# icdm-adteam/MoCoPCI

Hardware: AMD Instinct MI355X
Metric: interpolated frames/sec (higher is better)
Workload: dtype f32 (fused MLP layers: fp32 products as 6 bf16-MFMA partials of an exact 3-way split, fp32 accumulate; index paths exact f32)

## Files before the change

### mocopci_amd/csrc/cross.hip

```cpp
#include "common.h"
#include "cross_tile.h"

#ifdef MCP_CROSS_DIAG
__device__ unsigned long long g_cross_diag[8];
#define CROSS_STAMP(slot)                                                                            \
    do {                                                                                             \
        unsigned long long t_;                                                                       \
        __builtin_amdgcn_sched_barrier(0);                                                           \
        asm volatile("s_memtime %0\n\ts_waitcnt lgkmcnt(0)" : "=s"(t_)::"memory");                   \
        __builtin_amdgcn_sched_barrier(0);                                                           \
        if (blockIdx.x == 0 && blockIdx.y == 0 && threadIdx.x == 0) g_cross_diag[slot] += t_ - t_prev; \
        t_prev = t_;                                                                                 \
    } while (0)
#else
#define CROSS_STAMP(slot)
#endif

namespace {

constexpr int MAX_MAPPED_BATCH = 1024;

template <int CTRL>
__device__ __forceinline__ float dppf(float v) {
    return __uint_as_float(mcp_dpp<CTRL>(__float_as_uint(v)));
}
#define MCP_MAX_DPP(dst, src0, src1, CTRL)                                                                              \
    asm("s_nop 1\n\tv_max_f32_dpp %0, %1, %2 " CTRL : "+v"(dst) : "v"(src0), "v"(src1))

__device__ __forceinline__ float scatter_max(const f32x16 &acc, int lane) {
    float v8[8], v4[4], v2[2];
#pragma unroll
    for (int r = 0; r < 8; ++r) {
        const auto sw = __builtin_amdgcn_permlane16_swap(__float_as_uint(acc[r]), __float_as_uint(acc[r + 8]), false, false);
        const float a = __uint_as_float(sw[0]), b = __uint_as_float(sw[1]);
        asm("v_max_f32 %0, %1, %2" : "=v"(v8[r]) : "v"(a), "v"(b));
    }
#pragma unroll
    for (int r = 0; r < 4; ++r) {
        float d = v8[r + 4];
        MCP_MAX_DPP(d, v8[r], v8[r], "row_ror:8 row_mask:0xf bank_mask:0x3");
        MCP_MAX_DPP(d, v8[r + 4], d, "row_ror:8 row_mask:0xf bank_mask:0xc");
        v4[r] = d;
    }
#pragma unroll
    for (int r = 0; r < 2; ++r) {
        float d = v4[r + 2];
        MCP_MAX_DPP(d, v4[r], v4[r], "row_half_mirror row_mask:0xf bank_mask:0x5");
        MCP_MAX_DPP(d, v4[r + 2], d, "row_half_mirror row_mask:0xf bank_mask:0xa");
        v2[r] = d;
    }
    const bool b1 = (lane & 2) != 0;
    float keep = b1 ? v2[1] : v2[0];
    const float send = b1 ? v2[0] : v2[1];
    MCP_MAX_DPP(keep, send, keep, "quad_perm:[2,3,0,1] row_mask:0xf bank_mask:0xf");
    MCP_MAX_DPP(keep, keep, keep, "quad_perm:[1,0,3,2] row_mask:0xf bank_mask:0xf");
    return keep;
}
__device__ __forceinline__ int scatter_reg(int lane) { return ((lane >> 4) & 1) * 8 + ((lane >> 3) & 1) * 4 + ((lane >> 2) & 1) * 2 + ((lane >> 1) & 1); }

template <int D>
__global__ __launch_bounds__(256) void cross_pack_kernel(const float *__restrict__ wpos, const float *__restrict__ bpos,
                                                         const float *__restrict__ wmlp, const float *__restrict__ bmlp,
                                                         float *__restrict__ packed) {
    using L = CrossLds<D>;
    for (int e = blockIdx.x * 256 + threadIdx.x; e < L::FLOATS; e += gridDim.x * 256) {
        float v;
        if (e < L::OFF_POS) continue;
        else if (e < L::OFF_B) {
            const int f = e - L::OFF_POS, lane = f & 63, s = (f >> 6) & 1, t = f >> 7;
            const int row = 32 * t + (lane & 31), c = 2 * s + (lane >> 5);
            v = c < 3 ? wpos[row * 3 + c] : bpos[row];
        } else {
            const int f = e - L::OFF_B, r = f & 15, h = (f >> 4) & 1, t = f >> 5;
            v = bmlp[32 * t + mcp_chan_of(r, h)];
        }
        packed[e] = v;
    }
    mcp_split_weights(reinterpret_cast<uint4 *>(packed + L::OFF_W), wmlp, D, L::T, blockIdx.x * 256 + threadIdx.x, gridDim.x * 256);
}

template <int D>
struct CrossShape {
    static constexpr int NW = D == 128 ? 8 : 4;
    static constexpr int WG_PER_CU = D == 64 ? 3 : 1;
    static constexpr int GRID = D == 64 ? 768 : 256;
};

template <int D, int SPLIT>
__global__ __launch_bounds__(64 * CrossShape<D>::NW, CrossShape<D>::WG_PER_CU) void cross_kernel(long long total, int n1, int n2, const float *__restrict__ xyz1,
                                                           const float *__restrict__ xyz2, const float *__restrict__ points1,
                                                           const float *__restrict__ points2, const int *__restrict__ idx,
                                                           const int *__restrict__ idx2, const int *__restrict__ bmap, int shared,
                                                           const float *__restrict__ packed, float *__restrict__ out) {
    using L = CrossLds<D>;
    constexpr int T = L::T;
    constexpr int WAVES = CrossShape<D>::NW;
    constexpr int TO = T / SPLIT;
    constexpr int WH = L::W_FLOATS / SPLIT, SMALL = L::POS_FLOATS + L::B_FLOATS;
    extern __shared__ __attribute__((aligned(16))) float lds[];
    const int tid = threadIdx.x, split = blockIdx.y;
    static_assert(WH % 4 == 0 && SMALL % 4 == 0, "LDS image is copied as float4");
    for (int e = tid; e < WH / 4; e += 64 * WAVES)
        reinterpret_cast<float4 *>(lds)[e] = reinterpret_cast<const float4 *>(packed + L::OFF_W + (size_t)split * WH)[e];
    for (int e = tid; e < SMALL / 4; e += 64 * WAVES)
        reinterpret_cast<float4 *>(lds + WH)[e] = reinterpret_cast<const float4 *>(packed + L::OFF_POS)[e];
    if (bmap) {
        const int nb = (int)(total / n1);
        for (int e = tid; e < nb; e += 64 * WAVES) reinterpret_cast<int *>(lds + WH + SMALL + WAVES * D)[e] = bmap[e];
    }
    __syncthreads();

    const int lane = tid & 63, wave = tid >> 6, h = lane >> 5, col = lane & 31;
    const float *lpos = lds + WH, *lbias = lds + WH + L::POS_FLOATS;
    float *row1_lds = lds + WH + SMALL + wave * D;
    const int *bmap_lds = reinterpret_cast<const int *>(lds + WH + SMALL + WAVES * D);

#ifndef MCP_NO_XCD_MAP
    const bool by_xcd = gridDim.x >= 8 && (gridDim.x & 7) == 0;
#else
    const bool by_xcd = false;
#endif
    const long long chunk = by_xcd ? (total + 7) / 8 : total;
    const long long stride = (long long)(by_xcd ? gridDim.x >> 3 : gridDim.x) * WAVES;
    const long long limit = by_xcd ? min(total, ((long long)(blockIdx.x & 7) + 1) * chunk) : total;
    long long p = by_xcd ? (long long)(blockIdx.x & 7) * chunk + (long long)(blockIdx.x >> 3) * WAVES + wave : (long long)blockIdx.x * WAVES + wave;
    float q2x = 0.f, q2y = 0.f, q2z = 0.f, p1x = 0.f, p1y = 0.f, p1z = 0.f;
    float4 r1 = make_float4(0.f, 0.f, 0.f, 0.f);
    float4 rg[T][4];
    auto mapped = [&](int bb, int flag) -> long long { return (bmap && (shared & flag)) ? (long long)bmap_lds[bb] : (long long)bb; };
    struct Pos { int bb, off; };
    const int stride_b = (int)(stride / n1), stride_o = (int)(stride % n1);
    auto advance = [&](Pos q) {
        q.bb += stride_b;
        q.off += stride_o;
        if (q.off >= n1) { q.off -= n1; ++q.bb; }
        return q;
    };
    auto fetch = [&](long long pp, Pos q, int id) {
        const float *q2 = xyz2 + ((long long)q.bb * n2 + id) * 3;
        q2x = q2[0]; q2y = q2[1]; q2z = q2[2];
        p1x = xyz1[pp * 3 + 0]; p1y = xyz1[pp * 3 + 1]; p1z = xyz1[pp * 3 + 2];
        const float4 *row2 = reinterpret_cast<const float4 *>(points2 + (mapped(q.bb, 2) * n2 + id) * D);
        const float4 *row1 = reinterpret_cast<const float4 *>(points1 + (mapped(q.bb, 1) * n1 + q.off) * D);
        r1 = row1[lane < D / 4 ? lane : 0];
#pragma unroll
        for (int t = 0; t < T; ++t)
#pragma unroll
            for (int g = 0; g < 4; ++g) rg[t][g] = row2[(32 * t + 8 * g + 4 * h) >> 2];
    };
    auto nbr = [&](long long pp, Pos q) { return cross_nbr(idx, idx2, pp, [&] { return mapped(q.bb, 4) * n1 + q.off; }, col); };
    long long pn = p + stride;
    Pos qp{(int)(p / n1), (int)(p % n1)};
    Pos qn = advance(qp), qnn = advance(qn);
    int idn = 0;
    if (p < limit) {
        fetch(p, qp, nbr(p, qp));
        if (pn < limit) idn = nbr(pn, qn);
    }
#ifdef MCP_CROSS_DIAG
    unsigned long long t_prev = 0;
    CROSS_STAMP(7);
#endif
    for (; p < limit; p = pn, pn += stride) {
        CROSS_STAMP(0);
        McpSplit3 xs[2 * T];
        const float in0 = h ? q2y - p1y : q2x - p1x, in1 = h ? 1.0f : q2z - p1z;
        if (lane < D / 4) reinterpret_cast<float4 *>(row1_lds)[lane] = r1;
        __builtin_amdgcn_wave_barrier();
#pragma unroll
        for (int t = 0; t < T; ++t) {
            f32x16 acc;
#pragma unroll
            for (int g = 0; g < 4; ++g) {
                const float4 a = reinterpret_cast<const float4 *>(row1_lds)[(32 * t + 8 * g + 4 * h) >> 2];
                acc[4 * g + 0] = a.x; acc[4 * g + 1] = a.y; acc[4 * g + 2] = a.z; acc[4 * g + 3] = a.w;
            }
            acc = __builtin_amdgcn_mfma_f32_32x32x2f32(lpos[(t * 2 + 0) * 64 + lane], in0, acc, 0, 0, 0);
            acc = __builtin_amdgcn_mfma_f32_32x32x2f32(lpos[(t * 2 + 1) * 64 + lane], in1, acc, 0, 0, 0);
#pragma unroll
            for (int g = 0; g < 4; ++g) {
                acc[4 * g + 0] = leaky(acc[4 * g + 0] + rg[t][g].x);
                acc[4 * g + 1] = leaky(acc[4 * g + 1] + rg[t][g].y);
                acc[4 * g + 2] = leaky(acc[4 * g + 2] + rg[t][g].z);
                acc[4 * g + 3] = leaky(acc[4 * g + 3] + rg[t][g].w);
            }
            xs[2 * t + 0] = mcp_split_kstep(acc, 0);
            xs[2 * t + 1] = mcp_split_kstep(acc, 1);
        }
        __builtin_amdgcn_wave_barrier();
        CROSS_STAMP(1);
        if (pn < limit) {
            fetch(pn, qn, idn);
            if (pn + stride < limit) idn = nbr(pn + stride, qnn);
        }
        qn = qnn;
        qnn = advance(qnn);
        CROSS_STAMP(2);
#pragma unroll 1
        for (int tl = 0; tl < TO; ++tl) {
            const int t = TO * split + tl;
            f32x16 acc;
#pragma unroll
            for (int r = 0; r < 16; ++r) acc[r] = lbias[(t * 2 + h) * 16 + r];
            acc = mcp_tile_split<2 * T>(reinterpret_cast<const uint4 *>(lds) + (size_t)tl * (2 * T) * 3 * 64 + lane, xs, acc);
            CROSS_STAMP(3);
            const float m = leaky(scatter_max(acc, lane));
            if ((lane & 1) == 0) out[p * D + 32 * t + mcp_chan_of(scatter_reg(lane), h)] = m;
            CROSS_STAMP(4);
        }
    }
}

__global__ __launch_bounds__(64 * X256_WAVES, 1) void cross256_stream_kernel(long long total, int n1, int n2, const float *__restrict__ xyz1,
                                                                          const float *__restrict__ xyz2, const float *__restrict__ points1,
                                                                          const float *__restrict__ points2, const int *__restrict__ idx,
                                                                          const int *__restrict__ idx2, const int *__restrict__ bmap, int shared,
                                                                          const float *__restrict__ packed, float *__restrict__ out) {
    using L = CrossLds<256>;
    constexpr int D = 256, T = X256_T, WAVES = X256_WAVES, SMALL = L::POS_FLOATS + L::B_FLOATS;
    extern __shared__ __attribute__((aligned(16))) float lds[];
    uint4 *wbuf = reinterpret_cast<uint4 *>(lds);
    float *small = lds + 2 * X256_TILE_U4 * 4;
    float *row1_all = small + SMALL;
    int *bmap_lds = reinterpret_cast<int *>(row1_all + WAVES * D);
    const int tid = threadIdx.x, lane = tid & 63, wave = tid >> 6, h = lane >> 5, col = lane & 31;
    const uint4 *wimg = reinterpret_cast<const uint4 *>(packed + L::OFF_W);
    for (int e = tid; e < SMALL / 4; e += 64 * WAVES) reinterpret_cast<float4 *>(small)[e] = reinterpret_cast<const float4 *>(packed + L::OFF_POS)[e];
    if (bmap) {
        const int nb = (int)(total / n1);
        for (int e = tid; e < nb; e += 64 * WAVES) bmap_lds[e] = bmap[e];
    }
    for (int e = tid; e < X256_TILE_U4; e += 64 * WAVES) wbuf[e] = wimg[e];
    __syncthreads();
    const float *lpos = small, *lbias = small + L::POS_FLOATS;
    float *row1_lds = row1_all + wave * D;
    auto mapped = [&](int bb, int flag) -> long long { return (bmap && (shared & flag)) ? (long long)bmap_lds[bb] : (long long)bb; };

    const long long per_round = (long long)gridDim.x * WAVES;
    const long long first = (long long)blockIdx.x * WAVES;
    const int rounds = first < total ? (int)((total - first + per_round - 1) / per_round) : 0;
    int cur = 0;
    for (int g = 0; g < rounds; ++g) {
        const long long pw = first + (long long)g * per_round + wave;
        const bool live = pw < total;
        const long long p = live ? pw : total - 1;
        const int bb = (int)(p / n1), off = (int)(p - (long long)bb * n1);
        int id;
        if (!idx2) {
            id = idx[p * KNB + col];
        } else {
            const long long ps = mapped(bb, 4) * n1 + off;
            id = col >= 16 ? idx2[p * 16 + col - 16] : idx[ps * 16 + col];
        }
        const float *q2 = xyz2 + ((long long)bb * n2 + id) * 3;
        const float dx = q2[0] - xyz1[p * 3 + 0], dy = q2[1] - xyz1[p * 3 + 1], dz = q2[2] - xyz1[p * 3 + 2];
        const float in0 = h ? dy : dx, in1 = h ? 1.0f : dz;
        const float4 *row2 = reinterpret_cast<const float4 *>(points2 + (mapped(bb, 2) * n2 + id) * D);
        const float4 *row1 = reinterpret_cast<const float4 *>(points1 + (mapped(bb, 1) * n1 + off) * D);
        reinterpret_cast<float4 *>(row1_lds)[lane] = row1[lane];
        __builtin_amdgcn_wave_barrier();
        McpSplit3 xs[2 * T];
#pragma unroll
        for (int t = 0; t < T; ++t) {
            f32x16 acc;
            float4 rg[4];
#pragma unroll
            for (int gq = 0; gq < 4; ++gq) {
                const float4 a = reinterpret_cast<const float4 *>(row1_lds)[(32 * t + 8 * gq + 4 * h) >> 2];
                rg[gq] = row2[(32 * t + 8 * gq + 4 * h) >> 2];
                acc[4 * gq + 0] = a.x; acc[4 * gq + 1] = a.y; acc[4 * gq + 2] = a.z; acc[4 * gq + 3] = a.w;
            }
            acc = __builtin_amdgcn_mfma_f32_32x32x2f32(lpos[(t * 2 + 0) * 64 + lane], in0, acc, 0, 0, 0);
            acc = __builtin_amdgcn_mfma_f32_32x32x2f32(lpos[(t * 2 + 1) * 64 + lane], in1, acc, 0, 0, 0);
#pragma unroll
            for (int gq = 0; gq < 4; ++gq) {
                acc[4 * gq + 0] = leaky(acc[4 * gq + 0] + rg[gq].x);
                acc[4 * gq + 1] = leaky(acc[4 * gq + 1] + rg[gq].y);
                acc[4 * gq + 2] = leaky(acc[4 * gq + 2] + rg[gq].z);
                acc[4 * gq + 3] = leaky(acc[4 * gq + 3] + rg[gq].w);
            }
            xs[2 * t + 0] = mcp_split_kstep(acc, 0);
            xs[2 * t + 1] = mcp_split_kstep(acc, 1);
        }
        __builtin_amdgcn_wave_barrier();
#pragma unroll 1
        for (int t = 0; t < T; ++t) {
            const bool more = t + 1 < T || g + 1 < rounds;
            const uint4 *nsrc = wimg + (size_t)((t + 1) & (T - 1)) * X256_TILE_U4 + tid;
            uint4 nx[X256_TILE_U4 / (64 * X256_WAVES)];
#pragma unroll
            for (int i = 0; i < X256_TILE_U4 / (64 * WAVES); ++i) nx[i] = more ? nsrc[i * 64 * WAVES] : make_uint4(0u, 0u, 0u, 0u);
            f32x16 acc;
#pragma unroll
            for (int r = 0; r < 16; ++r) acc[r] = lbias[(t * 2 + h) * 16 + r];
            acc = mcp_tile_split<2 * T>(wbuf + (size_t)cur * X256_TILE_U4 + lane, xs, acc);
            const float m = leaky(scatter_max(acc, lane));
            if (live && (lane & 1) == 0) out[p * D + 32 * t + mcp_chan_of(scatter_reg(lane), h)] = m;
            uint4 *ndst = wbuf + (size_t)(cur ^ 1) * X256_TILE_U4 + tid;
#pragma unroll
            for (int i = 0; i < X256_TILE_U4 / (64 * WAVES); ++i) ndst[i * 64 * WAVES] = nx[i];
            __syncthreads();
            cur ^= 1;
        }
    }
}

int launch_cross256(long long total, int n1, int n2, const float *xyz1, const float *xyz2, const float *points1, const float *points2, const int *idx,
                    const int *idx2, const int *bmap, int shared, const float *packed, float *out, hipStream_t s) {
    const size_t lds = (size_t)(X256_LDS_FLOATS + (bmap ? MAX_MAPPED_BATCH : 0)) * sizeof(float);
    if (const int rc = mcp_allow_lds<cross256_stream_kernel>()) return rc;
    const long long want = (total + X256_WAVES - 1) / X256_WAVES;
    const unsigned grid = (unsigned)max(1LL, min(want, 256LL));
    hipLaunchKernelGGL(cross256_stream_kernel, dim3(grid), dim3(64 * X256_WAVES), lds, s, total, n1, n2, xyz1, xyz2, points1, points2, idx, idx2, bmap, shared,
                       packed, out);
    return mcp_launch_status();
}

template <int D, int SPLIT>
int launch_cross(long long total, int n1, int n2, const float *xyz1, const float *xyz2, const float *points1, const float *points2,
                 const int *idx, const int *idx2, const int *bmap, int shared, const float *packed, float *out, hipStream_t s) {
    using L = CrossLds<D>;
    constexpr int WAVES = CrossShape<D>::NW;
    const size_t lds = (L::W_FLOATS / SPLIT + L::POS_FLOATS + L::B_FLOATS + WAVES * D + (bmap ? MAX_MAPPED_BATCH : 0)) * sizeof(float);
    constexpr auto kern = cross_kernel<D, SPLIT>;
    if (const int rc = mcp_allow_lds<kern>()) return rc;
    const long long want = (total + WAVES * 8 - 1) / (WAVES * 8);
    const unsigned grid = (unsigned)max(1LL, min(want, (long long)(CrossShape<D>::GRID / SPLIT)));
    hipLaunchKernelGGL(kern, dim3(grid, SPLIT), dim3(64 * WAVES), lds, s, total, n1, n2, xyz1, xyz2, points1, points2, idx, idx2, bmap, shared, packed, out);
    return mcp_launch_status();
}

}

MCP_EXPORT int mcp_cross_packed_floats(int d) {
    return d == 64 ? CrossLds<64>::FLOATS : d == 128 ? CrossLds<128>::FLOATS : d == 256 ? CrossLds<256>::FLOATS : 0;
}

MCP_EXPORT int mcp_cross_pack(int d, const float *wpos, const float *bpos, const float *wmlp, const float *bmlp, float *packed,
                              mcp_stream_t stream) {
    MCP_CHECK_ARGS(wpos && bpos && wmlp && bmlp && packed);
    if (d != 64 && d != 128 && d != 256) return MCP_ERR_UNSUPPORTED;
    if (((uintptr_t)packed) & 15) return MCP_ERR_BAD_ARG;
    hipStream_t s = (hipStream_t)stream;
    if (d == 64) hipLaunchKernelGGL(cross_pack_kernel<64>, dim3(16), dim3(256), 0, s, wpos, bpos, wmlp, bmlp, packed);
    else if (d == 128) hipLaunchKernelGGL(cross_pack_kernel<128>, dim3(64), dim3(256), 0, s, wpos, bpos, wmlp, bmlp, packed);
    else hipLaunchKernelGGL(cross_pack_kernel<256>, dim3(256), dim3(256), 0, s, wpos, bpos, wmlp, bmlp, packed);
    return mcp_launch_status();
}

MCP_EXPORT int mcp_cross_volume(int b, int n1, int n2, int d, int k, const float *xyz1, const float *xyz2, const float *points1,
                                const float *points2, const int *idx, const int *idx2, const int *bmap, int shared, const float *packed, float *out,
                                mcp_stream_t stream) {
    MCP_CHECK_ARGS(b > 0 && n1 > 0 && n2 > 0 && xyz1 && xyz2 && points1 && points2 && idx && packed && out);
    if (k != KNB || (d != 64 && d != 128 && d != 256)) return MCP_ERR_UNSUPPORTED;
    if ((((uintptr_t)points1) | ((uintptr_t)points2) | ((uintptr_t)out) | ((uintptr_t)packed)) & 15) return MCP_ERR_BAD_ARG;
    if (bmap && b > MAX_MAPPED_BATCH) return MCP_ERR_UNSUPPORTED;
    hipStream_t s = (hipStream_t)stream;
    const long long total = (long long)b * n1;
    mcp_prof_begin(MCP_KERNEL_CROSS, s);
    const int rc = d == 64    ? launch_cross<64, 1>(total, n1, n2, xyz1, xyz2, points1, points2, idx, idx2, bmap, shared, packed, out, s)
                   : d == 128 ? launch_cross<128, 1>(total, n1, n2, xyz1, xyz2, points1, points2, idx, idx2, bmap, shared, packed, out, s)
                              : launch_cross256(total, n1, n2, xyz1, xyz2, points1, points2, idx, idx2, bmap, shared, packed, out, s);
    mcp_prof_end(MCP_KERNEL_CROSS, s);
    return rc;
}

#ifdef MCP_CROSS_DIAG
MCP_EXPORT int mcp_cross_diag_read(unsigned long long *out8) {
    hipError_t e = hipMemcpyFromSymbol(out8, HIP_SYMBOL(g_cross_diag), sizeof(unsigned long long) * 8);
    unsigned long long z[8] = {0};
    (void)hipMemcpyToSymbol(HIP_SYMBOL(g_cross_diag), z, sizeof(z));
    return (int)e;
}
#endif
```

### mocopci_amd/csrc/cross_tile.h

```cpp
#pragma once
#include "mfma_split.h"

namespace {

typedef float f32x16 __attribute__((ext_vector_type(16)));
constexpr int KNB = 32;
constexpr float SLOPE = 0.1f;
__device__ __forceinline__ float leaky(float v) { return mcp_max_raw(v, v * SLOPE); }

template <int D>
struct CrossLds {
    static constexpr int T = D / 32;
    static constexpr int W_FLOATS = T * (2 * T) * 3 * 64 * 4;
    static constexpr int POS_FLOATS = T * 2 * 64;
    static constexpr int B_FLOATS = T * 2 * 16;
    static constexpr int OFF_W = 0, OFF_POS = W_FLOATS, OFF_B = OFF_POS + POS_FLOATS;
    static constexpr int FLOATS = OFF_B + B_FLOATS;
};
__device__ __forceinline__ int cross_at(int t, int g, int h) { return (32 * t + 8 * g + 4 * h) >> 2; }

template <class PS>
__device__ __forceinline__ int cross_nbr(const int *idx, const int *idx2, long long p, PS ps, int col) {
    if (!idx2) return idx[p * KNB + col];
    const long long s = ps();
    return col >= 16 ? idx2[p * 16 + col - 16] : idx[s * 16 + col];
}
__device__ __forceinline__ int cross_nbr(const int *idx, const int *idx2, long long p, int col) {
    return cross_nbr(idx, idx2, p, [p] { return p; }, col);
}

template <class Own, class Gathered, class XSink>
__device__ __forceinline__ f32x16 cross_layer1(const float *pos, int t, int lane, float in0, float in1, Own own, Gathered gathered, XSink xsink) {
    f32x16 acc;
    float4 rg[4];
#pragma unroll
    for (int g = 0; g < 4; ++g) {
        const float4 a = own(g);
        rg[g] = gathered(g);
        acc[4 * g + 0] = a.x; acc[4 * g + 1] = a.y; acc[4 * g + 2] = a.z; acc[4 * g + 3] = a.w;
    }
    acc = __builtin_amdgcn_mfma_f32_32x32x2f32(pos[(t * 2 + 0) * 64 + lane], in0, acc, 0, 0, 0);
    acc = __builtin_amdgcn_mfma_f32_32x32x2f32(pos[(t * 2 + 1) * 64 + lane], in1, acc, 0, 0, 0);
#pragma unroll
    for (int g = 0; g < 4; ++g) {
        acc[4 * g + 0] = leaky(acc[4 * g + 0] + rg[g].x);
        acc[4 * g + 1] = leaky(acc[4 * g + 1] + rg[g].y);
        acc[4 * g + 2] = leaky(acc[4 * g + 2] + rg[g].z);
        acc[4 * g + 3] = leaky(acc[4 * g + 3] + rg[g].w);
        xsink(g, acc);
    }
    return acc;
}
struct CrossNoXSink {
    __device__ __forceinline__ void operator()(int, const f32x16 &) const {}
};

template <int CTRL>
__device__ __forceinline__ uint32_t max_dpp(uint32_t v) {
    const uint32_t o = mcp_dpp<CTRL>(v);
    return v > o ? v : o;
}
__device__ __forceinline__ uint32_t half_max_u32(uint32_t v) {
    v = max_dpp<0xB1>(v);
    v = max_dpp<0x4E>(v);
    v = max_dpp<0x141>(v);
    v = max_dpp<0x140>(v);
    const auto sw = __builtin_amdgcn_permlane16_swap(v, v, false, false);
    return sw[0] > sw[1] ? sw[0] : sw[1];
}
__device__ __forceinline__ bool cross_winner(float zv, int h, uint32_t lower_lanes) {
    const uint32_t key = mcp_ord(zv);
    const bool top = key == half_max_u32(key);
    const unsigned long long mask = __builtin_amdgcn_ballot_w64(top);
    const uint32_t mine = h ? (uint32_t)(mask >> 32) : (uint32_t)mask;
    return top && (mine & lower_lanes) == 0u;
}

constexpr int X256_T = CrossLds<256>::T, X256_KS = 2 * X256_T, X256_TILE_U4 = X256_KS * 3 * 64, X256_WAVES = 4;
constexpr int X256_SMALL = CrossLds<256>::POS_FLOATS + CrossLds<256>::B_FLOATS;
constexpr int X256_LDS_FLOATS = 2 * X256_TILE_U4 * 4 + X256_SMALL + X256_WAVES * 256;
static_assert(X256_T * X256_TILE_U4 * 4 == CrossLds<256>::W_FLOATS, "the tiles are the packed image's weight part");
static_assert((size_t)X256_LDS_FLOATS * sizeof(float) <= 160 * 1024, "LDS budget");

inline int cross_grad_check(int b, int n1, int n2, bool d_ok, int k, const float *xyz1, const float *xyz2, const float *points1, const float *points2,
                            const int *idx, const float *wpos, const float *bpos, const float *wmlp, const float *bmlp, const float *grad_out,
                            const float *grad_xyz1, const float *grad_dir, const float *grad_points1, const float *grad_rows, const float *grad_weights,
                            const void *workspace) {
    MCP_CHECK_ARGS(b > 0 && n1 > 0 && n2 > 0 && xyz1 && xyz2 && points1 && points2 && idx && wpos && bpos && wmlp && bmlp && grad_out && grad_xyz1 &&
                   grad_dir && grad_points1 && grad_rows && grad_weights && workspace);
    if (k != KNB || !d_ok) return MCP_ERR_UNSUPPORTED;
    if ((((uintptr_t)points1) | ((uintptr_t)points2) | ((uintptr_t)grad_out) | ((uintptr_t)grad_rows) | ((uintptr_t)workspace)) & 15) return MCP_ERR_BAD_ARG;
    return MCP_OK;
}

}
```

### mocopci_amd/csrc/mfma_split.h

```cpp
#pragma once
#include "common.h"

#ifndef MCP_SPLIT_SCHED_MASK
#define MCP_SPLIT_SCHED_MASK 0x0000
#endif

typedef float mcp_f32x16 __attribute__((ext_vector_type(16)));
typedef __bf16 mcp_bf16x8 __attribute__((ext_vector_type(8)));

__device__ __forceinline__ uint32_t mcp_top16(float x) { return __float_as_uint(x) & 0xFFFF0000u; }
__device__ __forceinline__ uint32_t mcp_pack_hi(float even, float odd) {
    return __builtin_amdgcn_perm(__float_as_uint(odd), __float_as_uint(even), 0x07060302u);
}

struct McpSplit3 {
    uint4 p1, p2, p3;
};
__device__ __forceinline__ McpSplit3 mcp_split8(const float *v) {
    float r1[8], r2[8];
#pragma unroll
    for (int i = 0; i < 8; ++i) {
        r1[i] = v[i] - __uint_as_float(mcp_top16(v[i]));
        r2[i] = r1[i] - __uint_as_float(mcp_top16(r1[i]));
    }
    McpSplit3 o;
#ifdef MCP_SPLIT_DIAG_NOSPLIT
    o.p1 = make_uint4(mcp_pack_hi(v[0], v[1]), mcp_pack_hi(v[2], v[3]), mcp_pack_hi(v[4], v[5]), mcp_pack_hi(v[6], v[7]));
    o.p2 = o.p1; o.p3 = o.p1;
    return o;
#endif
    o.p1 = make_uint4(mcp_pack_hi(v[0], v[1]), mcp_pack_hi(v[2], v[3]), mcp_pack_hi(v[4], v[5]), mcp_pack_hi(v[6], v[7]));
    o.p2 = make_uint4(mcp_pack_hi(r1[0], r1[1]), mcp_pack_hi(r1[2], r1[3]), mcp_pack_hi(r1[4], r1[5]), mcp_pack_hi(r1[6], r1[7]));
    o.p3 = make_uint4(mcp_pack_hi(r2[0], r2[1]), mcp_pack_hi(r2[2], r2[3]), mcp_pack_hi(r2[4], r2[5]), mcp_pack_hi(r2[6], r2[7]));
    return o;
}
__device__ __forceinline__ McpSplit3 mcp_split_kstep(const mcp_f32x16 &a, int s) {
    float v[8];
#pragma unroll
    for (int i = 0; i < 8; ++i) v[i] = a[8 * s + i];
    return mcp_split8(v);
}
__device__ __forceinline__ mcp_f32x16 mcp_mfma_bf16(uint4 a, uint4 b, mcp_f32x16 c) {
    return __builtin_amdgcn_mfma_f32_32x32x16_bf16(__builtin_bit_cast(mcp_bf16x8, a), __builtin_bit_cast(mcp_bf16x8, b), c, 0, 0, 0);
}
__device__ __forceinline__ mcp_f32x16 mcp_mfma_split(const uint4 *w, const McpSplit3 &x, mcp_f32x16 acc) {
    const uint4 w1 = w[0], w2 = w[64], w3 = w[128];
    acc = mcp_mfma_bf16(w3, x.p1, acc);
    acc = mcp_mfma_bf16(w1, x.p3, acc);
    acc = mcp_mfma_bf16(w2, x.p2, acc);
    acc = mcp_mfma_bf16(w2, x.p1, acc);
    acc = mcp_mfma_bf16(w1, x.p2, acc);
    acc = mcp_mfma_bf16(w1, x.p1, acc);
    return acc;
}
__device__ __forceinline__ void mcp_relu_split4(const mcp_f32x16 &a, int q, McpSplit3 &o) {
    float v[4], r1[4], r2[4];
#pragma unroll
    for (int i = 0; i < 4; ++i) {
        v[i] = fmaxf(a[4 * q + i], 0.f);
        r1[i] = v[i] - __uint_as_float(mcp_top16(v[i]));
        r2[i] = r1[i] - __uint_as_float(mcp_top16(r1[i]));
    }
    const uint32_t a1 = mcp_pack_hi(v[0], v[1]), b1 = mcp_pack_hi(v[2], v[3]);
    const uint32_t a2 = mcp_pack_hi(r1[0], r1[1]), b2 = mcp_pack_hi(r1[2], r1[3]);
    const uint32_t a3 = mcp_pack_hi(r2[0], r2[1]), b3 = mcp_pack_hi(r2[2], r2[3]);
    if (q & 1) { o.p1.z = a1; o.p1.w = b1; o.p2.z = a2; o.p2.w = b2; o.p3.z = a3; o.p3.w = b3; }
    else       { o.p1.x = a1; o.p1.y = b1; o.p2.x = a2; o.p2.y = b2; o.p3.x = a3; o.p3.y = b3; }
}
template <int NF, class Fill>
__device__ __forceinline__ mcp_f32x16 mcp_kstep_fill(const uint4 &w1, const uint4 &w2, const uint4 &w3, const McpSplit3 &x, mcp_f32x16 acc, Fill fill) {
    fill();
    acc = mcp_mfma_bf16(w3, x.p1, acc);
    acc = mcp_mfma_bf16(w1, x.p3, acc);
    acc = mcp_mfma_bf16(w2, x.p2, acc);
    acc = mcp_mfma_bf16(w2, x.p1, acc);
    acc = mcp_mfma_bf16(w1, x.p2, acc);
    acc = mcp_mfma_bf16(w1, x.p1, acc);
    if constexpr (NF > 0) {
        static_assert(NF <= 30, "at most five fillers per MFMA gap");
#define MCP_GAP(i)                                                                         \
    __builtin_amdgcn_sched_group_barrier(0x008, 1, 0);                                                                                    \
    if constexpr ((NF + 5 - (i)) / 6 > 0) __builtin_amdgcn_sched_group_barrier(0x002, (NF + 5 - (i)) / 6, 0);
        MCP_GAP(0) MCP_GAP(1) MCP_GAP(2) MCP_GAP(3) MCP_GAP(4) MCP_GAP(5)
#undef MCP_GAP
    }
    __builtin_amdgcn_sched_barrier(MCP_SPLIT_SCHED_MASK);
    return acc;
}
template <int KSTEPS>
__device__ __forceinline__ mcp_f32x16 mcp_tile_split(const uint4 *ws, const McpSplit3 *xs, mcp_f32x16 acc) {
    uint4 w1 = ws[0], w2 = ws[64], w3 = ws[128];
#pragma unroll
    for (int s = 0; s < KSTEPS; ++s) {
        uint4 n1 = w1, n2 = w2, n3 = w3;
#ifndef MCP_SPLIT_DIAG_NOLOAD
        if (s + 1 < KSTEPS) {
            const uint4 *nx = ws + (size_t)(s + 1) * 3 * 64;
            n1 = nx[0]; n2 = nx[64]; n3 = nx[128];
        }
#endif
        acc = mcp_mfma_bf16(w3, xs[s].p1, acc);
        acc = mcp_mfma_bf16(w1, xs[s].p3, acc);
        acc = mcp_mfma_bf16(w2, xs[s].p2, acc);
        acc = mcp_mfma_bf16(w2, xs[s].p1, acc);
        acc = mcp_mfma_bf16(w1, xs[s].p2, acc);
        acc = mcp_mfma_bf16(w1, xs[s].p1, acc);
        __builtin_amdgcn_sched_barrier(MCP_SPLIT_SCHED_MASK);
        w1 = n1; w2 = n2; w3 = n3;
    }
    return acc;
}

__device__ __forceinline__ void mcp_split_weights(uint4 *dst, const float *__restrict__ w, int cin, int out_tiles, int first, int stride) {
    const int ksteps = cin / 16;
    for (int e = first; e < out_tiles * ksteps * 64; e += stride) {
        const int lane = e & 63, s = (e >> 6) % ksteps, t = (e >> 6) / ksteps;
        float v[8];
#pragma unroll
        for (int i = 0; i < 8; ++i) v[i] = w[(size_t)(32 * t + (lane & 31)) * cin + 32 * (s >> 1) + mcp_chan_of(8 * (s & 1) + i, lane >> 5)];
        const McpSplit3 sp = mcp_split8(v);
        uint4 *o = dst + (size_t)(t * ksteps + s) * 3 * 64 + lane;
        o[0] = sp.p1;
        o[64] = sp.p2;
        o[128] = sp.p3;
    }
}
```

Before: 3645.

## Transpose cross MFMA output so each lane reduces its own row; raise grid caps

Swaps the MFMA operand order so the accumulator holds the transposed tile. The max over neighbours then becomes an in-register max3 chain plus a single permlane32 swap, replacing the multi-stage permlane16/DPP scatter reduction. A transposed bias table is added to the packed LDS image, and 32 lanes write contiguous output channels. Grid sizing also changes: the 256-wide kernel cap rises to 1024, the minimum points per wave becomes a tunable parameter, and env overrides are available behind MCP_AB. The extra bias table costs some LDS, which could reduce occupancy.

```diff
diff --git a/mocopci_amd/csrc/cross.hip b/mocopci_amd/csrc/cross.hip
--- a/mocopci_amd/csrc/cross.hip
+++ b/mocopci_amd/csrc/cross.hip
@@ -1,3 +1,5 @@
+#include <stdlib.h>
+
 #include "common.h"
 #include "cross_tile.h"
 
@@ -58,6 +60,22 @@
 }
 __device__ __forceinline__ int scatter_reg(int lane) { return ((lane >> 4) & 1) * 8 + ((lane >> 3) & 1) * 4 + ((lane >> 2) & 1) * 2 + ((lane >> 1) & 1); }
 
+__device__ __forceinline__ float row_max(const f32x16 &a) {
+    float m = __builtin_fmaxf(__builtin_fmaxf(a[0], a[1]), a[2]), t1, t2;
+    asm("v_max3_f32 %1, %3, %4, %5\n\t"
+        "v_max3_f32 %2, %6, %7, %8\n\t"
+        "v_max3_f32 %0, %0, %1, %2\n\t"
+        "v_max3_f32 %1, %9, %10, %11\n\t"
+        "v_max3_f32 %2, %12, %13, %14\n\t"
+        "v_max3_f32 %1, %1, %2, %15\n\t"
+        "v_max_f32 %0, %0, %1"
+        : "+v"(m), "=&v"(t1), "=&v"(t2)
+        : "v"(a[3]), "v"(a[4]), "v"(a[5]), "v"(a[6]), "v"(a[7]), "v"(a[8]), "v"(a[9]), "v"(a[10]), "v"(a[11]), "v"(a[12]), "v"(a[13]), "v"(a[14]),
+          "v"(a[15]));
+    const auto sw = __builtin_amdgcn_permlane32_swap(__float_as_uint(m), __float_as_uint(m), false, false);
+    return mcp_max_raw(__uint_as_float(sw[0]), __uint_as_float(sw[1]));
+}
+
 template <int D>
 __global__ __launch_bounds__(256) void cross_pack_kernel(const float *__restrict__ wpos, const float *__restrict__ bpos,
                                                          const float *__restrict__ wmlp, const float *__restrict__ bmlp,
@@ -70,9 +88,12 @@
             const int f = e - L::OFF_POS, lane = f & 63, s = (f >> 6) & 1, t = f >> 7;
             const int row = 32 * t + (lane & 31), c = 2 * s + (lane >> 5);
             v = c < 3 ? wpos[row * 3 + c] : bpos[row];
-        } else {
+        } else if (e < L::OFF_BT) {
             const int f = e - L::OFF_B, r = f & 15, h = (f >> 4) & 1, t = f >> 5;
             v = bmlp[32 * t + mcp_chan_of(r, h)];
+        } else {
+            const int f = e - L::OFF_BT, c = (f >> 2) & 31, t = f >> 9;
+            v = bmlp[32 * t + c];
         }
         packed[e] = v;
     }
@@ -84,7 +105,9 @@
     static constexpr int NW = D == 128 ? 8 : 4;
     static constexpr int WG_PER_CU = D == 64 ? 3 : 1;
     static constexpr int GRID = D == 64 ? 768 : 256;
+    static constexpr int MIN_PTS = 8;
 };
+constexpr long long X256_GRID_CAP = 1024;
 
 template <int D, int SPLIT>
 __global__ __launch_bounds__(64 * CrossShape<D>::NW, CrossShape<D>::WG_PER_CU) void cross_kernel(long long total, int n1, int n2, const float *__restrict__ xyz1,
@@ -96,7 +119,7 @@
     constexpr int T = L::T;
     constexpr int WAVES = CrossShape<D>::NW;
     constexpr int TO = T / SPLIT;
-    constexpr int WH = L::W_FLOATS / SPLIT, SMALL = L::POS_FLOATS + L::B_FLOATS;
+    constexpr int WH = L::W_FLOATS / SPLIT, SMALL = L::POS_FLOATS + L::B_FLOATS + L::BT_FLOATS;
     extern __shared__ __attribute__((aligned(16))) float lds[];
     const int tid = threadIdx.x, split = blockIdx.y;
     static_assert(WH % 4 == 0 && SMALL % 4 == 0, "LDS image is copied as float4");
@@ -111,7 +134,8 @@
     __syncthreads();
 
     const int lane = tid & 63, wave = tid >> 6, h = lane >> 5, col = lane & 31;
-    const float *lpos = lds + WH, *lbias = lds + WH + L::POS_FLOATS;
+    const float *lpos = lds + WH;
+    const float4 *lbias = reinterpret_cast<const float4 *>(lds + WH + L::POS_FLOATS + L::B_FLOATS) + col;
     float *row1_lds = lds + WH + SMALL + wave * D;
     const int *bmap_lds = reinterpret_cast<const int *>(lds + WH + SMALL + WAVES * D);
 
@@ -201,11 +225,14 @@
             const int t = TO * split + tl;
             f32x16 acc;
 #pragma unroll
-            for (int r = 0; r < 16; ++r) acc[r] = lbias[(t * 2 + h) * 16 + r];
-            acc = mcp_tile_split<2 * T>(reinterpret_cast<const uint4 *>(lds) + (size_t)tl * (2 * T) * 3 * 64 + lane, xs, acc);
+            for (int q = 0; q < 4; ++q) {
+                const float4 b = lbias[(t * 4 + q) * 32];
+                acc[4 * q + 0] = b.x; acc[4 * q + 1] = b.y; acc[4 * q + 2] = b.z; acc[4 * q + 3] = b.w;
+            }
+            acc = mcp_tile_split_t<2 * T>(reinterpret_cast<const uint4 *>(lds) + (size_t)tl * (2 * T) * 3 * 64 + lane, xs, acc);
             CROSS_STAMP(3);
-            const float m = leaky(scatter_max(acc, lane));
-            if ((lane & 1) == 0) out[p * D + 32 * t + mcp_chan_of(scatter_reg(lane), h)] = m;
+            const float m = leaky(row_max(acc));
+            if (lane < 32) out[p * D + 32 * t + col] = m;
             CROSS_STAMP(4);
         }
     }
@@ -305,12 +332,23 @@
     }
 }
 
+int grid_env(const char *name, int dflt) {
+#ifdef MCP_AB
+    const char *v = getenv(name);
+    return v && *v ? atoi(v) : dflt;
+#else
+    (void)name;
+    return dflt;
+#endif
+}
+
 int launch_cross256(long long total, int n1, int n2, const float *xyz1, const float *xyz2, const float *points1, const float *points2, const int *idx,
                     const int *idx2, const int *bmap, int shared, const float *packed, float *out, hipStream_t s) {
     const size_t lds = (size_t)(X256_LDS_FLOATS + (bmap ? MAX_MAPPED_BATCH : 0)) * sizeof(float);
     if (const int rc = mcp_allow_lds<cross256_stream_kernel>()) return rc;
     const long long want = (total + X256_WAVES - 1) / X256_WAVES;
-    const unsigned grid = (unsigned)max(1LL, min(want, 256LL));
+    static const long long cap = grid_env("MCP_CROSS256_GRID", X256_GRID_CAP);
+    const unsigned grid = (unsigned)max(1LL, min(want, cap));
     hipLaunchKernelGGL(cross256_stream_kernel, dim3(grid), dim3(64 * X256_WAVES), lds, s, total, n1, n2, xyz1, xyz2, points1, points2, idx, idx2, bmap, shared,
                        packed, out);
     return mcp_launch_status();
@@ -321,11 +359,13 @@
                  const int *idx, const int *idx2, const int *bmap, int shared, const float *packed, float *out, hipStream_t s) {
     using L = CrossLds<D>;
     constexpr int WAVES = CrossShape<D>::NW;
-    const size_t lds = (L::W_FLOATS / SPLIT + L::POS_FLOATS + L::B_FLOATS + WAVES * D + (bmap ? MAX_MAPPED_BATCH : 0)) * sizeof(float);
+    const size_t lds = (L::W_FLOATS / SPLIT + L::POS_FLOATS + L::B_FLOATS + L::BT_FLOATS + WAVES * D + (bmap ? MAX_MAPPED_BATCH : 0)) * sizeof(float);
     constexpr auto kern = cross_kernel<D, SPLIT>;
     if (const int rc = mcp_allow_lds<kern>()) return rc;
-    const long long want = (total + WAVES * 8 - 1) / (WAVES * 8);
-    const unsigned grid = (unsigned)max(1LL, min(want, (long long)(CrossShape<D>::GRID / SPLIT)));
+    static const long long cap = grid_env(D == 64 ? "MCP_CROSS64_GRID" : "MCP_CROSS128_GRID", CrossShape<D>::GRID);
+    static const long long min_pts = grid_env(D == 64 ? "MCP_CROSS64_MINPTS" : "MCP_CROSS128_MINPTS", CrossShape<D>::MIN_PTS);
+    const long long want = (total + WAVES * min_pts - 1) / (WAVES * min_pts);
+    const unsigned grid = (unsigned)max(1LL, min(want, cap / SPLIT));
     hipLaunchKernelGGL(kern, dim3(grid, SPLIT), dim3(64 * WAVES), lds, s, total, n1, n2, xyz1, xyz2, points1, points2, idx, idx2, bmap, shared, packed, out);
     return mcp_launch_status();
 }
diff --git a/mocopci_amd/csrc/cross_tile.h b/mocopci_amd/csrc/cross_tile.h
--- a/mocopci_amd/csrc/cross_tile.h
+++ b/mocopci_amd/csrc/cross_tile.h
@@ -14,8 +14,9 @@
     static constexpr int W_FLOATS = T * (2 * T) * 3 * 64 * 4;
     static constexpr int POS_FLOATS = T * 2 * 64;
     static constexpr int B_FLOATS = T * 2 * 16;
-    static constexpr int OFF_W = 0, OFF_POS = W_FLOATS, OFF_B = OFF_POS + POS_FLOATS;
-    static constexpr int FLOATS = OFF_B + B_FLOATS;
+    static constexpr int BT_FLOATS = D == 256 ? 0 : T * 4 * 32 * 4;
+    static constexpr int OFF_W = 0, OFF_POS = W_FLOATS, OFF_B = OFF_POS + POS_FLOATS, OFF_BT = OFF_B + B_FLOATS;
+    static constexpr int FLOATS = OFF_BT + BT_FLOATS;
 };
 __device__ __forceinline__ int cross_at(int t, int g, int h) { return (32 * t + 8 * g + 4 * h) >> 2; }
 
diff --git a/mocopci_amd/csrc/mfma_split.h b/mocopci_amd/csrc/mfma_split.h
--- a/mocopci_amd/csrc/mfma_split.h
+++ b/mocopci_amd/csrc/mfma_split.h
@@ -110,6 +110,29 @@
     }
     return acc;
 }
+template <int KSTEPS>
+__device__ __forceinline__ mcp_f32x16 mcp_tile_split_t(const uint4 *ws, const McpSplit3 *xs, mcp_f32x16 acc) {
+    uint4 w1 = ws[0], w2 = ws[64], w3 = ws[128];
+#pragma unroll
+    for (int s = 0; s < KSTEPS; ++s) {
+        uint4 n1 = w1, n2 = w2, n3 = w3;
+#ifndef MCP_SPLIT_DIAG_NOLOAD
+        if (s + 1 < KSTEPS) {
+            const uint4 *nx = ws + (size_t)(s + 1) * 3 * 64;
+            n1 = nx[0]; n2 = nx[64]; n3 = nx[128];
+        }
+#endif
+        acc = mcp_mfma_bf16(xs[s].p1, w3, acc);
+        acc = mcp_mfma_bf16(xs[s].p3, w1, acc);
+        acc = mcp_mfma_bf16(xs[s].p2, w2, acc);
+        acc = mcp_mfma_bf16(xs[s].p1, w2, acc);
+        acc = mcp_mfma_bf16(xs[s].p2, w1, acc);
+        acc = mcp_mfma_bf16(xs[s].p1, w1, acc);
+        __builtin_amdgcn_sched_barrier(MCP_SPLIT_SCHED_MASK);
+        w1 = n1; w2 = n2; w3 = n3;
+    }
+    return acc;
+}
 
 __device__ __forceinline__ void mcp_split_weights(uint4 *dst, const float *__restrict__ w, int cin, int out_tiles, int first, int stride) {
     const int ksteps = cin / 16;
```

New measurement: 3657, median of 3. Within noise of the previous version (+0.3%).
